# meteofrance/py4cast

Hardware: AMD Instinct MI355X
Metric: AR-training samples/sec (512x512x60 grid, 3-step rollout) (higher is better)
Workload: dtype bf16; 1 GPU; HalfUNet scaled_ar rollout T=3, grid 512x512x60 (+5 forcings, 4 statics), WeightedLoss(MSE), AdamW, B=2/GPU; global_batch=2, parallelism=dp1, border_size=0, setup_steps=2, accumulate_grad_batches=1, hip_graph=False, deterministic_library_solvers=False, full=False

## Files before the change

### include/py4cast_hip.h

```cpp
#ifndef PY4CAST_HIP_H
#define PY4CAST_HIP_H

#include <stddef.h>
#include <stdint.h>

#ifdef __cplusplus
extern "C" {
#endif

#define P4C_VERSION 100

typedef void* p4c_stream_t;

enum p4c_error {
    P4C_OK = 0,
    P4C_ERR_INVALID = -1,
    P4C_ERR_LAUNCH = -2,
    P4C_ERR_RUNTIME = -3,
    P4C_ERR_UNSUPPORTED = -4
};

enum p4c_dtype { P4C_F32 = 0, P4C_BF16 = 1 };

enum p4c_loss_kind { P4C_LOSS_MSE = 0, P4C_LOSS_L1 = 1 };
// ... 351 lines not shown
    int32_t cout;
    int32_t dx_channels;
    int32_t dtype;
    int32_t norm;
    int32_t groups;
    int32_t has_bias;
    float eps;
    float momentum;
    int32_t compute;
    int32_t weights_prepared;
    int32_t skip_out_conv;
} p4c_halfunet_desc;

int p4c_first_conv_tail_slots(int B, int H, int W);
int p4c_first_conv_tail(const void* x, int x_cs, int cin, const float* w, void* y, float* stat_partial, int B, int H, int W, p4c_stream_t stream);

int p4c_set_side_stream(p4c_stream_t side, void* const* events, int n_events);
int p4c_side_stream_defer(int on);
int p4c_side_stream_enable(int on);
long long p4c_side_stream_launch_count(void);
int p4c_side_stream_join(p4c_stream_t stream);
int p4c_graph_replace_memsets(void* graph, int* replaced, int* left);

int64_t p4c_halfunet_param_count(const p4c_halfunet_desc* d);
int p4c_halfunet_workspace_bytes(const p4c_halfunet_desc* d, size_t* saved_bytes, size_t* scratch_bytes);
typedef struct p4c_halfunet_layout_t {
    int64_t elem_bytes;
    int64_t Y[12], P[5], S, norm[12], saved_bytes;
    int64_t G0, TB, DY[2][12], k1[2][12], k2[2][12], scratch_bytes;
    int64_t w[12], gamma[12], beta[12], wout, params_bytes;
// ... 280 lines not shown
```

### py4cast_amd/_lib_model.py

```python

import ctypes
from ctypes import c_float, c_int, c_int32, c_int64, c_size_t, c_void_p

P, I, L, F = c_void_p, c_int, c_int64, c_float


class HalfUNetDesc(ctypes.Structure):

    _fields_ = [
        ("B", c_int32), ("H", c_int32), ("W", c_int32),
        ("cin", c_int32), ("cin_pad", c_int32), ("cout", c_int32), ("dx_channels", c_int32),
        ("dtype", c_int32), ("norm", c_int32), ("groups", c_int32), ("has_bias", c_int32),
        ("eps", c_float), ("momentum", c_float), ("compute", c_int32),
        ("weights_prepared", c_int32), ("skip_out_conv", c_int32),
    ]


DP = ctypes.POINTER(HalfUNetDesc)


class HalfUNetLayout(ctypes.Structure):

    _fields_ = [
        ("elem_bytes", c_int64),
# ... 28 lines not shown

SIGNATURES = {
    "p4c_prep_weights": [P, I, I, I, I, I, I, P, I, P],
    "p4c_conv_fwd": [P, I, I, I, P, I, P, P, I, P, P, I, P, I, I, I, I, P],
    "p4c_conv_wgrad": [P, I, I, I, I, P, P, I, P, I, I, P, P, I, I, I, P],
    "p4c_conv_small_fwd": [P, I, I, I, P, I, P, P, I, P, P, I, P, I, I, I, I, P, P, P, P, P, P, P, P, P, P, P, P, F, F, P, P, P, P, P, P,
                           P, P, P, P, P, P, P, P, P],
    "p4c_norm_finalize": [P, I, I, L, I, I, P, P, F, F, P, P, P, P, P, P, P],
    "p4c_conv_fwd_compact": [P, I, P, I, P, I, I, I, I, P],
    "p4c_conv_wgrad_compact": [P, I, I, P, I, I, I, P, P, I, I, I, P],
    "p4c_conv_wgrad_nb": [P, P, P, I, P, P, P, P, P, P, P, P, P, I, I, P, P, I, I, I, P],
    "p4c_conv_wgrad_kernel_kind": [I, I, I, I],
    "p4c_out_conv_bwd": [P, P, P, P, P, P, P, P, P, I, P, P, I, L, P],
    "p4c_upsample_sum_bwd_x": [I, P, I, I, I, P, P, P, P, P],
    "p4c_first_conv_tail": [P, I, I, P, P, P, I, I, I, P],
    "p4c_halfunet_workspace_bytes": [DP, ctypes.POINTER(c_size_t), ctypes.POINTER(c_size_t)],
    "p4c_halfunet_layout": [DP, ctypes.POINTER(HalfUNetLayout)],
    "p4c_halfunet_prepare_weights": [DP, P, P, P],
    "p4c_halfunet_forward": [DP, P, P, P, P, P, P, I, P],
    "p4c_halfunet_tail": [DP, P, P, P, P, P, P],
    "p4c_halfunet_backward": [DP, P, P, P, P, P, P, P, I, P],
    "p4c_side_stream_defer": [I],
    "p4c_side_stream_enable": [I],
    "p4c_side_stream_join": [P],
    "p4c_edge_gather_add_fwd": [P, P, P, P, P, P, L, I, I, I, P],
    "p4c_edge_gather_add_bwd": [P, P, P, P, P, P, P, L, I, I, I, P],
    "p4c_segment_sum": [P, P, P, P, P, L, L, I, I, I, P],
    "p4c_segment_sum_pair": [P, P, P, P, L, P, P, P, L, L, I, I, P],
    "p4c_row_layernorm_fwd": [P, P, P, P, F, P, L, I, I, P],
    "p4c_row_layernorm_bwd": [P, P, P, F, P, P, P, P, L, I, I, P],
# ... 55 lines not shown
    "p4c_deeplab_assemble_bwd": [P, P, P, P, P, I, I, I, P],
    "p4c_up2_cat_fwd": [P, P, P, L, I, I, I, I, I, P],
    "p4c_up2_cat_bwd": [P, L, P, P, I, I, I, I, I, P],
    "p4c_customunet_stem_fwd": [P, P, P, P, L, P, P, I, I, I, I, P],
    "p4c_customunet_stem_bwd": [P, P, L, P, P, P, P, P, P, P, P, I, I, I, I, P],
    "p4c_dlp_dw3x3_fwd": [P, P, P, P, P, I, I, I, I, I, I, I, I, P],
    "p4c_dlp_dw3x3_dgrad": [P, P, P, P, P, I, I, I, I, I, I, I, I, P],
    "p4c_dlp_dw3x3_wgrad": [P, P, P, P, P, I, I, I, I, I, I, I, I, P],
    "p4c_dlp_up_cat_fwd": [P, P, P, L, I, I, I, I, I, I, P],
    "p4c_dlp_up_cat_bwd": [P, L, P, P, I, I, I, I, I, I, P],
}
OTHER = {
    "p4c_conv_wgrad_workspace_bytes": ([I, I], c_size_t),
    "p4c_out_conv_bwd_slots": ([I, L], c_int),
    "p4c_first_conv_tail_slots": ([I, I, I], c_int),
    "p4c_out_conv_bwd_workspace_bytes": ([I, L], c_size_t),
    "p4c_conv_stat_tiles": ([I, I, I, I, I, I], c_int),
    "p4c_conv_stat_tiles_ks": ([I, I, I, I, I, I, I], c_int),
    "p4c_conv_kernel_kind": ([I, I, I, I, I, I, I], c_int),
    "p4c_conv_small_ok": ([I, I, I, I], c_int),
    "p4c_conv_small_stat_slots": ([I, I, I], c_int),
    "p4c_conv_compact_supported": ([I, I, I, I, I, I], c_int),
    "p4c_halfunet_param_count": ([DP], c_int64),
    "p4c_window_attn_bwd_workspace_bytes": ([I, I, I, I, I], c_size_t),
    "p4c_row_layernorm_bwd_workspace_bytes": ([L, I, I], c_size_t),
    "p4c_row_linear_wgrad_workspace_bytes": ([L, I], c_size_t),
    "p4c_row_gemm_supported": ([I, I], c_int),
    "p4c_row_gemm_wgrad_supported": ([I, I, I], c_int),
    "p4c_row_gemm_wgrad_workspace_bytes": ([L, I, I, I], c_size_t),
    "p4c_row_mlp_bwd_workspace_bytes": ([L, I], c_size_t),
# ... 17 lines not shown
```

### py4cast_amd/csrc/conv_bf16.hip

```cpp
#include <stdlib.h>

#include <type_traits>

#include "kernels.hpp"

namespace p4c {

typedef float f32x16 __attribute__((ext_vector_type(16)));
typedef float f32x4 __attribute__((ext_vector_type(4)));
typedef __bf16 bf16x8 __attribute__((ext_vector_type(8)));
typedef __bf16 bf16x4 __attribute__((ext_vector_type(4)));
typedef short s16x4 __attribute__((ext_vector_type(4)));

constexpr int BTW = 32;

#ifndef P4C_PRIO
#define P4C_PRIO 0
#endif
#ifndef P4C_EXP
#define P4C_EXP 0
#endif

#ifdef P4C_STAMPS
__device__ unsigned long long* g_stamps = nullptr;
// ... 2150 lines not shown
    if (blockIdx.x == 0 && blockIdx.y == 0 && (int)threadIdx.x < pb.n_zero) pb.zero_words[threadIdx.x] = 0u;
    const PrepJob& jb = pb.job[blockIdx.y];
    const int total = jb.M_pad * jb.K_pad * jb.ntaps;
    const int kv = pb.bf16 ? 8 : 4;
    const int ksteps = jb.K_pad / (2 * kv);
    for (int i = blockIdx.x * 256 + threadIdx.x; i < total; i += gridDim.x * 256) {
        int t = i;
        const int j = t % kv; t /= kv;
        const int m_l = t & 63; t >>= 6;
        const int h = t & 1; t >>= 1;
        const int ks = t % ksteps; t /= ksteps;
        const int tap = t % jb.ntaps;
        const int mb = t / jb.ntaps;
        const int k = 2 * kv * ks + kv * h + j, m = 64 * mb + m_l;
        float v = 0.0f;
        if (!jb.transpose_flip) {
            if (m < jb.CO && k < jb.CI) v = jb.w[((int64_t)m * jb.CI + k) * jb.ntaps + tap];
        } else {
            if (k < jb.CO && m < jb.CI) v = jb.w[((int64_t)k * jb.CI + m) * jb.ntaps + (jb.ntaps - 1 - tap)];
        }
        if (pb.bf16) reinterpret_cast<__bf16*>(jb.out)[i] = (__bf16)v;
        else reinterpret_cast<float*>(jb.out)[i] = v;
    }
}

int prep_weights_batch(const PrepBatch& pb, hipStream_t stream) {
    if (pb.n <= 0) return P4C_OK;
    int maxtotal = 0;
    for (int i = 0; i < pb.n; ++i) {
        const int t = pb.job[i].M_pad * pb.job[i].K_pad * pb.job[i].ntaps;
        if (t > maxtotal) maxtotal = t;
// ... 10 lines not shown
```

### py4cast_amd/csrc/conv_rows.hip

```cpp
#include <stddef.h>
#include <stdlib.h>

#include "kernels.hpp"

namespace p4c {

#ifndef P4C_EXP
#define P4C_EXP 0
#endif

#ifdef P4C_STAMPS
__device__ unsigned long long* g_rows_stamps = nullptr;
__device__ __forceinline__ void rows_stamp(int slot) {
    if (g_rows_stamps && blockIdx.x == 7 && blockIdx.y == 0 && blockIdx.z == 0 && (threadIdx.x & 63) == 0) {
        unsigned long long t;
        asm volatile("s_memtime %0\n\ts_waitcnt lgkmcnt(0)" : "=s"(t)::"memory");
        g_rows_stamps[2 * slot] = t;
        g_rows_stamps[2 * slot + 1] = __builtin_amdgcn_s_memrealtime();
    }
}
#define P4C_STAMP(slot) rows_stamp(slot)
#if P4C_STAMPS == 1
#define P4C_STAMP_ROW(slot) rows_stamp(slot)
#else
// ... 55 lines not shown
    const float ylo = __builtin_bit_cast(float, y2 << 16), yhi = __builtin_bit_cast(float, y2 & 0xffff0000u);
    const float glo = __builtin_fmaf(ylo, sc.x, sh.x) > 0.f ? __builtin_bit_cast(float, a2 << 16) : 0.f;
    const float ghi = __builtin_fmaf(yhi, sc.y, sh.y) > 0.f ? __builtin_bit_cast(float, a2 & 0xffff0000u) : 0.f;
    const float lo = __builtin_fmaf(al.x, glo, __builtin_fmaf(be.x, ylo, de.x));
    const float hi = __builtin_fmaf(al.y, ghi, __builtin_fmaf(be.y, yhi, de.y));
    const f32x2 v = {lo, hi};
    return __builtin_bit_cast(unsigned int, __builtin_convertvector(v, bf16x2));
}

__device__ __forceinline__ __amdgpu_buffer_rsrc_t make_rsrc(const void* base, unsigned int bytes) {
    return __builtin_amdgcn_make_buffer_rsrc(const_cast<void*>(base), 0, (int)bytes, 0x00020000);
}

__device__ __forceinline__ void lds_barrier() { asm volatile("s_waitcnt lgkmcnt(0)\n\ts_barrier" ::: "memory"); }

template <bool HP, bool HQ, bool HS>
__device__ __forceinline__ void conv_row(const bf16x8 (&A)[9][4], f32x16& P, f32x16& Q, f32x16& S, bf16x8 (&fb)[6],
                                         const char* rb, const char* rbn, bool pf, char* stg, const int (&soff)[4]) {
    using namespace rows;
    constexpr int PIXB = Lay<32>::PIXB;
    auto stage = [&](int g) __attribute__((always_inline)) {
        const f32x2 lo = {P[4 * g], P[4 * g + 1]}, hi = {P[4 * g + 2], P[4 * g + 3]};
        u32x2 o;
        o[0] = __builtin_bit_cast(unsigned int, __builtin_convertvector(lo, bf16x2));
        o[1] = __builtin_bit_cast(unsigned int, __builtin_convertvector(hi, bf16x2));
        *reinterpret_cast<u32x2*>(stg + soff[g]) = o;
    };
#pragma unroll
    for (int s = 0; s < 14; ++s) {
        const int o = s + 3;
        if (!(P4C_EXP & 16)) {
            if (o < 12) {
                fb[o % 6] = *reinterpret_cast<const bf16x8*>(rb + (o >> 2) * PIXB + (o & 3) * 32);
            } else if (o < 15) {
                if (pf) fb[o % 6] = *reinterpret_cast<const bf16x8*>(rbn + ((o - 12) >> 2) * PIXB + ((o - 12) & 3) * 32);
            }
            __builtin_amdgcn_sched_barrier(0);
            if (HP && s < 12) {
                P = __builtin_amdgcn_mfma_f32_32x32x16_bf16(A[6 + (s >> 2)][s & 3], fb[s % 6], P, 0, 0, 0);
                __builtin_amdgcn_sched_barrier(0);
            }
        }
        if (s >= 2) {
            const int q = s - 2;
            if (HQ && !(P4C_EXP & 16)) {
                Q = __builtin_amdgcn_mfma_f32_32x32x16_bf16(A[3 + (q >> 2)][q & 3], fb[q % 6], Q, 0, 0, 0);
                __builtin_amdgcn_sched_barrier(0);
            }
            if (HP && s >= 12) { stage(2 * (s - 12)); __builtin_amdgcn_sched_barrier(0); }
            if (HS && !(P4C_EXP & 16)) {
                if (q == 0) {
                    f32x16 z;
#pragma unroll
                    for (int i = 0; i < 16; ++i) z[i] = 0.f;
                    S = __builtin_amdgcn_mfma_f32_32x32x16_bf16(A[q >> 2][q & 3], fb[q % 6], z, 0, 0, 0);
                } else {
                    S = __builtin_amdgcn_mfma_f32_32x32x16_bf16(A[q >> 2][q & 3], fb[q % 6], S, 0, 0, 0);
                }
                __builtin_amdgcn_sched_barrier(0);
            }
            if (HP && s >= 12) { stage(2 * (s - 12) + 1); __builtin_amdgcn_sched_barrier(0); }
        }
    }
}

struct Acc16 { f32x4 v[2][2]; };

template <bool HP, bool HQ, bool HS>
__device__ __forceinline__ void conv_row16(const bf16x8 (&A)[9][2][2], Acc16& P, Acc16& Q, Acc16& S, bf16x8 (&fb)[6],
                                           int (&boff)[3][2], int delta, bool pf, const char* lring, char* stg,
                                           const int (&soff)[2]) {
    auto stage = [&](int mb, int nb) __attribute__((always_inline)) {
        const f32x4 a = P.v[mb][nb];
        const f32x2 lo = {a[0], a[1]}, hi = {a[2], a[3]};
        u32x2 o;
        o[0] = __builtin_bit_cast(unsigned int, __builtin_convertvector(lo, bf16x2));
// ... 55 lines not shown
    NormBwdCoef nb;
    BatchFin fin;
};
template <typename T>
__device__ __forceinline__ T late_arg(size_t offset) {
#if defined(__HIP_DEVICE_COMPILE__)
    const char* ka = (const char*)__builtin_amdgcn_kernarg_segment_ptr();
    asm volatile("" : "+s"(ka));
    return *reinterpret_cast<const T*>(ka + offset);
#else
    (void)offset;
    return T{};
#endif
}

template <int MODE, bool BST, int MF, int KS, bool CPT = false, int IV = 4>
__global__ void __launch_bounds__(512) __attribute__((amdgpu_waves_per_eu(2, 2)))
    conv3x3_bf16_rows_kernel(RowsArgs args) {
    static_assert(!CPT || (MODE == 0 && !BST && MF == 32), "compact channels: plain launches only");
    static_assert(IV == 4 || IV == 2, "rows per interval");
    using namespace rows;
    constexpr int NLD = (IV * ROWSLOTS + 255) / 256, NST = IV * 2;
    const __bf16* __restrict__ in = args.in;
    const __bf16* __restrict__ wp = args.wp;
    const float* __restrict__ in_scale = args.in_scale;
    const float* __restrict__ in_shift = args.in_shift;
    __bf16* __restrict__ out = args.out;
    float* __restrict__ stat_partial = args.stat_partial;
    const int out_cs = args.out_cs, H = args.H, W = args.W, rows_lo = args.rows_lo, rows_rem = args.rows_rem;
    const RingBwdStats& bst = args.bst;
    const NormBwdCoef& nb = args.nb;
    typedef Lay<MF> LY;
    constexpr int PIXB = LY::PIXB, RROW = LY::RROW, RINGB = LY::RINGB;
    extern __shared__ __attribute__((aligned(16))) char smem[];
    char* lring = smem;
    char* lstg = smem + RINGB;

// ... 2 lines not shown
    const int seg = blockIdx.x, strip = blockIdx.y, b = blockIdx.z;
    const int nseg = gridDim.x, nstrips = gridDim.y;
    const int wg_id = (b * nstrips + strip) * nseg + seg, wg_count = nseg * nstrips * gridDim.z;
    const int y0 = seg * rows_lo + (seg < rows_rem ? seg : rows_rem);
    const int R = rows_lo + (seg < rows_rem ? 1 : 0);
    const int x0 = strip * SW;
    const int K = (R + 2 + IV - 1) / IV;

    if (wv >= 4) {
        const int ltid = threadIdx.x - 256, lwv = wv - 4, c8 = ltid & 7;
        const int ipb = CPT ? args.in_cs * 2 : 128;
        const bool in_ch = !CPT || 8 * c8 < args.in_cs, out_ch = !CPT || 8 * c8 < out_cs;
        const __amdgpu_buffer_rsrc_t rs_in = make_rsrc(in + (int64_t)b * H * W * (ipb >> 1), (unsigned int)H * W * (unsigned int)ipb);
        const __amdgpu_buffer_rsrc_t rs_out = make_rsrc(out + (int64_t)b * H * W * out_cs, (unsigned int)H * W * out_cs * 2u);
        int gofs[NLD], lofs[NLD], lim[NLD];
        int rr = 0, rem = ltid;
#pragma unroll
        for (int it = 0; it < NLD; ++it) {
            const int idx = ltid + it * 256;
            if (it > 0) { rem += 256; if (rem >= ROWSLOTS) { rem -= ROWSLOTS; ++rr; } }
            const int col = rem >> 3;
            gofs[it] = in_ch ? (rr * W + col) * ipb + 16 * c8 : OOB;
            lofs[it] = rr * RROW + LY::slot_off(col, c8);
            lim[it] = ((unsigned)(x0 - 1 + col) < (unsigned)W) ? idx : OOB;
        }
        {
            const int left = x0 == 0 ? 1 : 0;
            const int c_hi = W - x0 + 1 < LW ? W - x0 + 1 : LW;
            const int ninv = left + (LW - c_hi);
            for (int rz = 0; rz < NR; ++rz)
                for (int j = ltid; j < ninv * 8; j += 256) {
                    const int s8 = j & 7, ci = j >> 3;
                    const int col = (left && ci == 0) ? 0 : c_hi + ci - left;
                    *reinterpret_cast<u32x4*>(lring + rz * RROW + col * PIXB + 16 * s8) = u32x4{0u, 0u, 0u, 0u};
                }
        }
        int dofs[NST], sofs[NST];
#pragma unroll
        for (int j = 0; j < NST; ++j) {
            const int px = (ltid + j * 256) >> 3, row = px >> 6, col = px & 63;
            dofs[j] = out_ch ? ((row * W + col) * out_cs + 8 * c8) * 2 : OOB;
            sofs[j] = row * SROW + col * 128 + ((c8 ^ ((col >> 1) & 7)) << 4);
        }
        f32x2 sc[4], sh[4], al[4], be[4], dl[4];
#pragma unroll
        for (int k = 0; k < 4; ++k) {
            sc[k] = sh[k] = al[k] = be[k] = dl[k] = f32x2{0.f, 0.f};
            if (MODE == 2 || MODE == 3) {
                sc[k] = *reinterpret_cast<const f32x2*>(in_scale + b * 64 + 8 * c8 + 2 * k);
// ... 19 lines not shown
            const int m0 = IV * k;
            int nrows = R + 2 - m0;
            nrows = nrows > IV ? IV : (nrows < 0 ? 0 : nrows);
            if ((P4C_EXP & 2) && k > 1) nrows = 0;
            const int nact = nrows * ROWSLOTS;
            const int gy0 = y0 - 1 + m0, gx0 = x0 - 1;
            if (gy0 >= 0 && gy0 + nrows <= H) {
                const int so = (gy0 * W + gx0) * ipb;
#pragma unroll
                for (int it = 0; it < NLD; ++it)
                    im.s[it] = __builtin_amdgcn_raw_buffer_load_b128(rs_in, (lim[it] < nact) ? gofs[it] : OOB, so, 0);
                if (MODE == 4) {
#pragma unroll
                    for (int it = 0; it < NLD; ++it)
                        ty.s[it] = __builtin_amdgcn_raw_buffer_load_b128(rs_nby, (lim[it] < nact) ? gofs[it] : OOB, so, 0);
                }
            } else {
#pragma unroll
                for (int it = 0; it < NLD; ++it) {
                    const int idx = ltid + it * 256, rr = idx / ROWSLOTS;
                    const int gy = gy0 + rr, gx = gx0 + ((idx - rr * ROWSLOTS) >> 3);
                    const bool ok = (idx < nact) & ((unsigned)gy < (unsigned)H) & ((unsigned)gx < (unsigned)W) & in_ch;
                    im.s[it] = __builtin_amdgcn_raw_buffer_load_b128(rs_in, ok ? (gy * W + gx) * ipb + 16 * c8 : OOB, 0, 0);
                    if (MODE == 4) ty.s[it] = __builtin_amdgcn_raw_buffer_load_b128(rs_nby, ok ? (gy * W + gx) * 128 + 16 * c8 : OOB, 0, 0);
                }
            }
        };
        auto store = [&](const Img& im, int k) __attribute__((always_inline)) {
            const int m0 = IV * k;
            int nrows = R + 2 - m0;
// ... 272 lines not shown
        {
            const char* wsrc = reinterpret_cast<const char*>(wp) + (h * 64 + ct * 32 + r) * 16;
#pragma unroll
            for (int tap = 0; tap < 9; ++tap)
#pragma unroll
                for (int ks = 0; ks < 4; ++ks) A[tap][ks] = *reinterpret_cast<const bf16x8*>(wsrc + (tap * 4 + ks) * 2048);
        }
        const int lane_base = (32 * ph + r) * PIXB + 16 * h;
        int soff[4];
#pragma unroll
        for (int g = 0; g < 4; ++g) soff[g] = (32 * ph + r) * 128 + 8 * h + (((4 * ct + g) ^ (((32 * ph + r) >> 1) & 7)) << 4);
        f32x16 a, bq, c;
#pragma unroll
        for (int i = 0; i < 16; ++i) a[i] = bq[i] = c[i] = 0.f;
        bf16x8 fb[6];
        auto rbase = [&](int mm) __attribute__((always_inline)) { return lring + (mm & 7) * RROW + lane_base; };
        auto issue3 = [&](const char* rb) __attribute__((always_inline)) {
            if (!(P4C_EXP & 16)) {
#pragma unroll
                for (int o = 0; o < 3; ++o) fb[o] = *reinterpret_cast<const bf16x8*>(rb + (o >> 2) * PIXB + (o & 3) * 32);
            }
        };
        if (wv == 0) P4C_STAMP(10);
        lds_barrier();
        if (wv == 0) P4C_STAMP(11);
        issue3(rbase(0));
#define P4C_ROW(HP, HQ, HS, P, Q, S)                                                                                        \
    {                                                                                                                       \
        const bool pf = ((m & (IV - 1)) != IV - 1) && (m != last);                                                          \
        if (wv == 0) P4C_STAMP_ROW(300 + 2 * m);                                                                            \
        conv_row<HP, HQ, HS>(A, P, Q, S, fb, rbase(m), rbase(m + 1), pf, lstg + (m & 7) * SROW, soff);                     \
        if (wv == 0) P4C_STAMP_ROW(301 + 2 * m);                                                                            \
        if (m == last) {                                                                                                    \
            P4C_STAMP(700 + 8 * (m >> 2) + 2 * wv);                                                                         \
            lds_barrier();                                                                                                  \
            P4C_STAMP(701 + 8 * (m >> 2) + 2 * wv);                                                                         \
        } else if ((m & (IV - 1)) == IV - 1) {                                                                              \
            P4C_STAMP(700 + 8 * (m >> 2) + 2 * wv);                                                                         \
            lds_barrier();                                                                                                  \
            P4C_STAMP(701 + 8 * (m >> 2) + 2 * wv);                                                                         \
            issue3(rbase(m + 1));                                                                                           \
        }                                                                                                                   \
        ++m;                                                                                                                \
    }
        P4C_ROW(false, false, true, a, a, a)
        P4C_ROW(false, true, true, a, a, bq)
// ... 79 lines not shown
#define P4C_ROTATE() { const Acc16 t_ = a; a = bq; bq = c; c = t_; }
        while (m < R) {
            P4C_ROW(true, true, true, a, bq, c)
            P4C_ROTATE()
        }
        P4C_ROW(true, true, false, a, bq, a)
        P4C_ROTATE()
        P4C_ROW(true, false, false, a, a, a)
#undef P4C_ROTATE
#undef P4C_ROW
        if (P4C_EXP & 16) { asm volatile("" ::"v"(A[0][0][0]), "v"(A[8][1][1])); }
    }
    if (wv == 0) P4C_STAMP(12);
}

static int rows_mfma_shape() {
    const char* e = diag_env("P4C_ROWS_MFMA");
    return (e && atoi(e) == 16) ? 16 : 32;
}

template <int MODE, bool BST, int KS, int IV = 4>
int launch_rows_mode(const __bf16* in, const __bf16* wp, const float* in_scale, const float* in_shift, __bf16* out, int out_cs,
                     float* stat_partial, int B, int H, int W, int nstrips, int nseg, hipStream_t stream, const BatchFin& fin,
                     const RingBwdStats& bst, const NormBwdCoef& nb = NormBwdCoef{}) {
    const RowsArgs args{in, wp, in_scale, in_shift, out, stat_partial, out_cs, H, W, H / nseg, H % nseg, fin.slots ? 1 : 0, 64, bst, nb, fin};
    if (KS == 1 || MODE == 4 || rows_mfma_shape() == 32) {
        P4C_TRY(ensure_dyn_smem((const void*)conv3x3_bf16_rows_kernel<MODE, BST, 32, KS, false, IV>, rows::Lay<32>::SMEM));
        hipLaunchKernelGGL((conv3x3_bf16_rows_kernel<MODE, BST, 32, KS, false, IV>), dim3(nseg, nstrips, B), dim3(512), rows::Lay<32>::SMEM, stream, args);
    } else if (KS == 3 && MODE != 4) {
        constexpr int M16 = MODE == 4 ? 0 : MODE;
// ... 81 lines not shown
    const int rc = ks == 3 ? launch_rows_compact<3>((const __bf16*)in, in_cs, (const __bf16*)wp, (__bf16*)out, out_cs, B, H, W, nstrips, nseg, stream)
                           : launch_rows_compact<1>((const __bf16*)in, in_cs, (const __bf16*)wp, (__bf16*)out, out_cs, B, H, W, nstrips, nseg, stream);
    if (rc != P4C_OK) return rc;
    P4C_CHECK_LAUNCH("conv_bf16_rows_compact");
    return P4C_OK;
}

int launch_conv_bf16_rows_wide_pixels(const void* in, int pixel_channels, const void* wp, void* out, int B, int H, int W, hipStream_t stream) {
    if (pixel_channels < 64 || pixel_channels % 8 || !conv_bf16_is_rows(P4C_BF16, 64, 3, 1, 64, B, H, W) ||
        (int64_t)H * W * pixel_channels * 2 >= (int64_t)1 << 31)
        return fail(P4C_ERR_UNSUPPORTED, "conv_bf16_rows_wide_pixels: unsupported shape (%d-channel pixels, %dx%dx%d)", pixel_channels, B, H, W);
    int nstrips, nseg;
    conv_rows_geometry(B, H, W, &nstrips, &nseg);
    const int rc = launch_rows_compact<3>((const __bf16*)in, pixel_channels, (const __bf16*)wp, (__bf16*)out, 64, B, H, W, nstrips, nseg, stream);
    if (rc != P4C_OK) return rc;
    P4C_CHECK_LAUNCH("conv_bf16_rows_wide_pixels");
    return P4C_OK;
}

int conv_rows_stat_slots(int B, int H, int W) {
    int nstrips, nseg;
    conv_rows_geometry(B, H, W, &nstrips, &nseg);
    return nstrips * nseg * 4;
}

int launch_conv3x3_bf16_rows(const void* inv, const void* wpv, int ks, const float* in_scale, const float* in_shift, int in_relu,
                             void* outv, int out_cs, float* stat_partial, int B, int H, int W, hipStream_t stream, const BatchFin* finp,
                             const RingBwdStats* bst, int* nblk_out, const NormBwdCoef* nb) {
    const __bf16* in = (const __bf16*)inv;
    const __bf16* wp = (const __bf16*)wpv;
    __bf16* out = (__bf16*)outv;
// ... 27 lines not shown
```

### py4cast_amd/csrc/conv_thin.hip

```cpp
#include <stdlib.h>

#include "kernels.hpp"

namespace p4c {
namespace {

typedef float f32x16 __attribute__((ext_vector_type(16)));
typedef float f32x4 __attribute__((ext_vector_type(4)));
typedef __bf16 bf16x8 __attribute__((ext_vector_type(8)));
typedef unsigned int u32x4 __attribute__((ext_vector_type(4)));

constexpr int OOB = 0x7fffffff;
constexpr int SP = 68;
constexpr int WIMG_BYTES = 2 * 5 * 64 * 16;

struct ThinArgs {
    const __bf16* x;
    const float* w;
    __bf16* y;
    float* stat_partial;
    int x_cs, c0, nc, cin;
    int H, W, nblk;
};

// ... 115 lines not shown
    if (n > 256) n = 256;
    const int64_t cap = 2 * (int64_t)num_cus() / (B > 0 ? B : 1);
    if (n > cap && cap >= 1) n = cap;
    return n < 1 ? 1 : (int)n;
}

}

bool first_conv_split_ok(int compute, int storage, int cin, int cin_pad, int B, int H, int W) {
    const char* e = diag_env("P4C_FIRST_CONV_SPLIT");
    if (e && e[0] == '0') return false;
    return compute == P4C_BF16 && storage == P4C_BF16 && cin_pad == 96 && cin > 64 && cin <= 72 && W % 32 == 0 &&
           conv_bf16_is_rows(storage, 64, 3, 1, 64, B, H, W) && (int64_t)H * W * 192 < ((int64_t)1 << 31);
}

int first_conv_tail_slots(int B, int H, int W) { return tail_blocks(B, H, W) * 4; }

int launch_first_conv_tail(const void* x, int x_cs, int cin, const float* w, void* y, float* stat_partial, int B, int H, int W, hipStream_t stream) {
    ThinArgs a{(const __bf16*)x, w, (__bf16*)y, stat_partial, x_cs, 64, cin - 64, cin, H, W, tail_blocks(B, H, W)};
    hipLaunchKernelGGL(first_conv_tail_kernel, dim3(a.nblk, B), dim3(256), 0, stream, a);
    P4C_CHECK_LAUNCH("first_conv_tail");
    return P4C_OK;
}

namespace {
namespace wt {
constexpr int SW = 64, LW = SW + 2;
constexpr int RPI = 2;
constexpr int NRX = 8, NRD = 2 * RPI;
constexpr int XROW = LW * 16, DROW = SW * 128;
constexpr int XRING = NRX * XROW, DRING = NRD * DROW;
constexpr int SLAB = 9 * 8 * 64;
__device__ __forceinline__ int slot_off(int col, int c8) { return col * 128 + ((((c8 >> 2) ^ (col >> 1)) & 1) << 6) + ((c8 & 3) << 4); }
}

// ... 177 lines not shown
    P4C_CHECK_LAUNCH("conv3x3_wgrad_thin_bf16");
    *nslots_out = nwg;
    return P4C_OK;
}

}

extern "C" int p4c_first_conv_tail_slots(int B, int H, int W) { return p4c::first_conv_tail_slots(B, H, W); }
extern "C" int p4c_first_conv_tail(const void* x, int x_cs, int cin, const float* w, void* y, float* stat_partial, int B, int H, int W,
                                   p4c_stream_t stream) {
    P4C_CHECK_ARG(x && w && y, "p4c_first_conv_tail: NULL pointer");
    P4C_CHECK_ARG(cin > 64 && cin <= 72 && x_cs >= 72 && x_cs % 8 == 0 && W % 32 == 0 && B > 0 && H > 0,
                  "p4c_first_conv_tail: 65..72 input channels on pixels of >= 72 channels (multiple of 8), W a multiple of 32");
    return p4c::launch_first_conv_tail(x, x_cs, cin, w, y, stat_partial, B, H, W, p4c::as_stream(stream));
}
```

### py4cast_amd/csrc/halfunet.cpp

```cpp
#include <stdlib.h>

#include <atomic>
#include <functional>
#include <vector>

#include "kernels.hpp"

namespace p4c {
namespace {

constexpr int NF = 64;
constexpr int NLEV = 5;
constexpr int NCONV = 12;
constexpr int NWSLOT = 2 * NCONV + 3;

constexpr int64_t HANDOFF_SLOT_FLOATS = 256 * 128;

struct Layout {
    int esz;
    int64_t n[NLEV];
    int Hk[NLEV], Wk[NLEV];
    int64_t w[NCONV], gamma[NCONV], beta[NCONV], wout, nparams;
    int64_t Y[NCONV], P[NLEV], S, act_elems, norm_base, norm[NCONV], saved_bytes;
    int64_t wslot_floats;
// ... 150 lines not shown
}

inline void* wslot(const WS& ws, int slot) { return ws.f(ws.L.wprep + (int64_t)slot * ws.L.wslot_floats); }

int prepare_weights(const p4c_halfunet_desc& d, const WS& ws, const float* params, int which, hipStream_t st) {
    const Layout& L = ws.L;
    PrepBatch pb;
    pb.n = 0;
    pb.bf16 = d.compute == P4C_BF16;
    for (int i = 0; i < NCONV; ++i) {
        if (which & 1) pb.job[pb.n++] = {params + L.w[i], wslot(ws, i), NF, conv_cin(d, i), 9, 0, 64, conv_cin_pad(d, i)};
        if (which & 2) pb.job[pb.n++] = {params + L.w[i], wslot(ws, NCONV + i), NF, conv_cin(d, i), 9, 1, i == 0 ? 64 * dx_blocks(d) : 64, NF};
    }
    if (which & 1) pb.job[pb.n++] = {params + L.wout, wslot(ws, 2 * NCONV), d.cout, NF, 1, 0, 64, NF};
    if ((which & 1) && first_conv_split_ok(d.compute, d.dtype, d.cin, d.cin_pad, d.B, d.H, d.W))
        pb.job[pb.n++] = {params + L.w[0], wslot(ws, 2 * NCONV + 2), NF, d.cin, 9, 0, 64, NF};
    if (which & 2) pb.job[pb.n++] = {params + L.wout, wslot(ws, 2 * NCONV + 1), d.cout, NF, 1, 1, 64, NF};
    pb.zero_words = reinterpret_cast<unsigned int*>(ws.f(L.tickets));
    pb.n_zero = 64;
    return prep_weights_batch(pb, st);
}

bool small_handoff(const p4c_halfunet_desc& d, const Layout& L, int lev, int training) {
    const char* ie = diag_env("P4C_NO_INKERNEL_FINALIZE");
    return lev > 0 && training && d.norm == 0 && d.compute == P4C_BF16 && !(ie && ie[0] == '1') &&
           conv_small_handoff_ok(d.dtype, d.B, L.Hk[lev], L.Wk[lev]);
}

int conv_block_fwd(const p4c_halfunet_desc& d, const WS& ws, int i, const void* in, const Norm* in_norm, const float* params,
                   float* running, int training, hipStream_t st, int handoff = 0) {
    const Layout& L = ws.L;
// ... 21 lines not shown
    if (small) {
        float* other = statp ? statp + HANDOFF_SLOT_FLOATS : nullptr;
        BatchFin pre{};
        if (handoff == 2) {
            Norm pn = norm_at(ws, i - 1, d.B);
            float* prm = running ? running + (int64_t)(i - 1) * 128 : nullptr;
            pre = BatchFin{other, nullptr, params + L.gamma[i - 1], params + L.beta[i - 1], prm, prm ? prm + 64 : nullptr,
                           pn.scale, pn.shift, pn.mean, pn.rstd, (double)d.B * H * W, d.eps, d.momentum, d.B};
        }
        const bool given = in_norm && handoff != 2;
        P4C_TRY(launch_conv3x3_bf16_small(in, wp, given ? in_norm->scale : nullptr, given ? in_norm->shift : nullptr, in_norm ? 1 : 0,
                                          ws.act(L.Y[i]), handoff == 1 ? other : statp, d.B, H, W, st,
                                          infin && handoff != 1 ? &fin : nullptr, handoff == 2 ? &pre : nullptr));
        if (handoff == 1) return P4C_OK;
        ntiles = conv_small_stat_slots(d.B, H, W);
    } else if (i == 0 && !in_norm && first_conv_split_ok(d.compute, d.dtype, d.cin, d.cin_pad, d.B, H, W)) {
        P4C_TRY(launch_conv_bf16_rows_wide_pixels(in, d.cin_pad, wslot(ws, 2 * NCONV + 2), ws.act(L.Y[i]), d.B, H, W, st));
        P4C_TRY(launch_first_conv_tail(in, d.cin_pad, d.cin, params + L.w[0], ws.act(L.Y[i]), statp, d.B, H, W, st));
        ntiles = first_conv_tail_slots(d.B, H, W);
    } else {
        P4C_TRY(conv_fwd(d.compute, d.dtype, in, conv_cin_pad(d, i), wp, 3, in_norm ? in_norm->scale : nullptr,
                         in_norm ? in_norm->shift : nullptr, in_norm ? 1 : 0, ws.act(L.Y[i]), NF, statp, d.B, H, W, 1, st,
                         infin ? &fin : nullptr));
    }
    if (infin) return P4C_OK;
    if (batch_stats) {
        P4C_TRY(norm_finalize(statp, ntiles, d.B, (int64_t)H * W, d.norm,
                              d.groups, params + L.gamma[i], params + L.beta[i], d.eps, d.momentum,
                              d.norm == 0 ? rm : nullptr, d.norm == 0 ? rv : nullptr, nm.scale, nm.shift, nm.mean, nm.rstd, st));
    } else {
// ... 613 lines not shown
```

### py4cast_amd/csrc/kernels.hpp

```cpp
#pragma once
#include "common.hpp"

namespace p4c {

int prep_weights(const float* w, int CO, int CI, int ks, int transpose_flip, int M_pad, int K_pad, float* out,
                 hipStream_t stream);
int conv_fwd_f32(const float* in, int CI, const float* wp, int ks, const float* in_scale, const float* in_shift,
                 int in_relu, const float* bias, float* out, int out_cs, float* stat_partial, int B, int H, int W,
                 int m_blocks, hipStream_t stream);
int conv_wgrad_f32(const float* in, int CI, int ks, const float* in_scale, const float* in_shift, int in_relu,
                   const float* dout, float* partial, int G, int B, int H, int W, int CO, int CIreal, float* grad,
                   hipStream_t stream);
static inline int64_t wgrad_partial_floats(int CI_pad, int ks, int G) { return (int64_t)2 * G * ks * ks * CI_pad * 64; }

int wgrad_reduce(const float* partial, int nslots, int ks, int CI_pad, int ci_lo, int ci_hi, int CO, int CI, float* grad,
                 hipStream_t stream, int ci_base = 0);
struct WgradReduceJob {
    const float* partial;
    float* grad;
    int nslots, ntaps, CI_pad, ci_lo, ci_hi, CO, CI;
    int ci_base = 0;
};
constexpr int WGRAD_BATCH_MAX = 24;
struct WgradCollect {
    WgradReduceJob job[WGRAD_BATCH_MAX];
    int n = 0;
};
void wgrad_collect_into(WgradCollect* c);
int wgrad_reduce_batch(const WgradCollect& c, hipStream_t stream);

int prep_weights_bf16(const float* w, int CO, int CI, int ks, int transpose_flip, int M_pad, int K_pad, void* out,
                      hipStream_t stream);
struct PrepJob {
    const float* w;
    void* out;
    int CO, CI, ntaps, transpose_flip, M_pad, K_pad;
};
struct PrepBatch {
    PrepJob job[32];
    int n;
    int bf16;
    unsigned int* zero_words;
    int n_zero;
};

struct BatchFin {
    float* slots;
    unsigned int* ticket;
    const float* gamma;
    const float* beta;
    float* running_mean;
// ... 72 lines not shown
bool conv_wgrad_bf16_takes_nb(int storage, int CI, int ks, int B);
bool conv_rows_compact_ok(int storage, int in_cs, int out_cs, int ks, int B, int H, int W);
int launch_conv_bf16_rows_compact(const void* in, int in_cs, const void* wp, int ks, void* out, int out_cs, int B, int H, int W,
                                  hipStream_t stream);
int conv_wgrad_bf16_compact(const void* in, int in_cs, int ks, const void* dout, int dout_cs, float* partial, int G, int B, int H, int W,
                            int CO, int CIreal, float* grad, hipStream_t stream);

bool first_conv_split_ok(int compute, int storage, int cin, int cin_pad, int B, int H, int W);
int first_conv_tail_slots(int B, int H, int W);
int launch_first_conv_tail(const void* x, int x_cs, int cin, const float* w, void* y, float* stat_partial, int B, int H, int W, hipStream_t stream);
bool conv_wgrad_thin_ok(int storage, int in_cs, int ci_real, int dout_cs, int ks, int B, int H, int W);
int conv_wgrad_thin_slots(int G, int B, int H, int W, int* nseg_out = nullptr);
int launch_conv3x3_wgrad_thin_bf16(const void* x, int in_cs, const void* dout, float* partial, int G, int B, int H, int W, hipStream_t stream,
                                   int* nslots_out);
int launch_conv_bf16_rows_wide_pixels(const void* in, int pixel_channels, const void* wp, void* out, int B, int H, int W, hipStream_t stream);

int norm_finalize(const float* partial, int tiles_per_sample, int B, int64_t hw, int mode, int groups, const float* gamma,
                  const float* beta, float eps, float momentum, float* running_mean, float* running_var, float* scale,
                  float* shift, float* mean, float* rstd, hipStream_t stream);
int norm_eval(int B, const float* gamma, const float* beta, float eps, const float* running_mean,
              const float* running_var, float* scale, float* shift, float* mean, float* rstd, hipStream_t stream);
int norm_bwd_blocks(int64_t hw);
int norm_bwd(int storage, const void* dA, const void* y, const float* scale, const float* shift, const float* mean,
             const float* rstd, const float* gamma, int relu, int B, int64_t hw, int mode, int groups, int training,
             float* partial, float* k1, float* k2, float* dgamma, float* dbeta, void* dY, hipStream_t stream, int pre_nblk = 0,
             unsigned int* fin_ticket = nullptr, bool pre_finalized = false);
constexpr int NORM_BWD_MAX_BLOCKS = 1024;
int pool_fwd(int storage, const void* y, const float* scale, const float* shift, int B, int H, int W, void* P,
             hipStream_t stream);
int upsum_fwd(int storage, const void* const* y, const float* const* scale, const float* const* shift, int B, int H, int W,
// ... 28 lines not shown
```

Baseline: 457.3 samples/s.

## Fold first-conv tail channels into the rows MFMA kernel as a ninth octet

Adds a thin variant of the compact 3x3 rows conv kernel that also loads the ninth 8-channel octet of input pixels and runs extra MFMAs on a packed weight image, so the first HalfUNet conv (65..72 input channels) runs in a single launch. Previously it ran as a wide-pixel rows conv over 64 channels plus a separate tail kernel that re-read the input and accumulated the rest. Weight prep gains a thin packing mode and extra LDS is reserved for the tail weights. This removes one launch and a second pass over input and output, at the cost of more LDS, more registers and a longer per-row schedule in the hot kernel. The new path is taken by default and can be disabled through an environment variable.

```diff
diff --git a/include/py4cast_hip.h b/include/py4cast_hip.h
--- a/include/py4cast_hip.h
+++ b/include/py4cast_hip.h
@@ -389,6 +389,10 @@
 
 int p4c_first_conv_tail_slots(int B, int H, int W);
 int p4c_first_conv_tail(const void* x, int x_cs, int cin, const float* w, void* y, float* stat_partial, int B, int H, int W, p4c_stream_t stream);
+int p4c_first_conv_one_slots(int B, int H, int W);
+int p4c_first_conv_one(const void* x, int x_cs, int cin, const float* w, void* y, float* stat_partial, int B, int H, int W, p4c_stream_t stream);
+int p4c_first_conv_two(const void* x, int x_cs, int cin, const float* w, void* y, float* stat_partial, int B, int H, int W, p4c_stream_t stream);
+long long p4c_first_conv_launch_count(void);
 
 int p4c_set_side_stream(p4c_stream_t side, void* const* events, int n_events);
 int p4c_side_stream_defer(int on);
diff --git a/py4cast_amd/_lib_model.py b/py4cast_amd/_lib_model.py
--- a/py4cast_amd/_lib_model.py
+++ b/py4cast_amd/_lib_model.py
@@ -66,6 +66,8 @@
     "p4c_out_conv_bwd": [P, P, P, P, P, P, P, P, P, I, P, P, I, L, P],
     "p4c_upsample_sum_bwd_x": [I, P, I, I, I, P, P, P, P, P],
     "p4c_first_conv_tail": [P, I, I, P, P, P, I, I, I, P],
+    "p4c_first_conv_one": [P, I, I, P, P, P, I, I, I, P],
+    "p4c_first_conv_two": [P, I, I, P, P, P, I, I, I, P],
     "p4c_halfunet_workspace_bytes": [DP, ctypes.POINTER(c_size_t), ctypes.POINTER(c_size_t)],
     "p4c_halfunet_layout": [DP, ctypes.POINTER(HalfUNetLayout)],
     "p4c_halfunet_prepare_weights": [DP, P, P, P],
@@ -151,6 +153,8 @@
     "p4c_conv_wgrad_workspace_bytes": ([I, I], c_size_t),
     "p4c_out_conv_bwd_slots": ([I, L], c_int),
     "p4c_first_conv_tail_slots": ([I, I, I], c_int),
+    "p4c_first_conv_one_slots": ([I, I, I], c_int),
+    "p4c_first_conv_launch_count": ([], ctypes.c_longlong),
     "p4c_out_conv_bwd_workspace_bytes": ([I, L], c_size_t),
     "p4c_conv_stat_tiles": ([I, I, I, I, I, I], c_int),
     "p4c_conv_stat_tiles_ks": ([I, I, I, I, I, I, I], c_int),
diff --git a/py4cast_amd/csrc/conv_bf16.hip b/py4cast_amd/csrc/conv_bf16.hip
--- a/py4cast_amd/csrc/conv_bf16.hip
+++ b/py4cast_amd/csrc/conv_bf16.hip
@@ -2188,7 +2188,10 @@
         const int mb = t / jb.ntaps;
         const int k = 2 * kv * ks + kv * h + j, m = 64 * mb + m_l;
         float v = 0.0f;
-        if (!jb.transpose_flip) {
+        if (jb.thin) {
+            const int ky = tap >> 1, kx = 2 * (tap & 1) + h;
+            if (kx < 3 && m < jb.CO && 64 + j < jb.CI) v = jb.w[((int64_t)m * jb.CI + 64 + j) * 9 + 3 * ky + kx];
+        } else if (!jb.transpose_flip) {
             if (m < jb.CO && k < jb.CI) v = jb.w[((int64_t)m * jb.CI + k) * jb.ntaps + tap];
         } else {
             if (k < jb.CO && m < jb.CI) v = jb.w[((int64_t)k * jb.CI + m) * jb.ntaps + (jb.ntaps - 1 - tap)];
diff --git a/py4cast_amd/csrc/conv_rows.hip b/py4cast_amd/csrc/conv_rows.hip
--- a/py4cast_amd/csrc/conv_rows.hip
+++ b/py4cast_amd/csrc/conv_rows.hip
@@ -93,11 +93,14 @@
 
 __device__ __forceinline__ void lds_barrier() { asm volatile("s_waitcnt lgkmcnt(0)\n\ts_barrier" ::: "memory"); }
 
-template <bool HP, bool HQ, bool HS>
+template <bool HP, bool HQ, bool HS, bool THIN = false>
 __device__ __forceinline__ void conv_row(const bf16x8 (&A)[9][4], f32x16& P, f32x16& Q, f32x16& S, bf16x8 (&fb)[6],
-                                         const char* rb, const char* rbn, bool pf, char* stg, const int (&soff)[4]) {
+                                         const char* rb, const char* rbn, bool pf, char* stg, const int (&soff)[4],
+                                         const char* tw = nullptr, int tl0 = 0, int tl1 = 0) {
     using namespace rows;
     constexpr int PIXB = Lay<32>::PIXB;
+    bf16x8 tb[2], ta[2];
+    auto thin_has = [](int j) { return j % 3 == 0 ? HP : (j % 3 == 1 ? HQ : HS); };
     auto stage = [&](int g) __attribute__((always_inline)) {
         const f32x2 lo = {P[4 * g], P[4 * g + 1]}, hi = {P[4 * g + 2], P[4 * g + 3]};
         u32x2 o;
@@ -114,6 +117,12 @@
             } else if (o < 15) {
                 if (pf) fb[o % 6] = *reinterpret_cast<const bf16x8*>(rbn + ((o - 12) >> 2) * PIXB + ((o - 12) & 3) * 32);
             }
+            if constexpr (THIN) {
+                if (s == 3) tb[0] = *reinterpret_cast<const bf16x8*>(rb + tl0);
+                if (s == 6) tb[1] = *reinterpret_cast<const bf16x8*>(rb + tl1);
+                if (s >= 3 && s < 9 && thin_has(s - 3))
+                    ta[(s - 3) & 1] = *reinterpret_cast<const bf16x8*>(tw + ((2 - (s - 3) % 3) * 2 + (s - 3) / 3) * 2048);
+            }
             __builtin_amdgcn_sched_barrier(0);
             if (HP && s < 12) {
                 P = __builtin_amdgcn_mfma_f32_32x32x16_bf16(A[6 + (s >> 2)][s & 3], fb[s % 6], P, 0, 0, 0);
@@ -139,6 +148,14 @@
                 __builtin_amdgcn_sched_barrier(0);
             }
             if (HP && s >= 12) { stage(2 * (s - 12) + 1); __builtin_amdgcn_sched_barrier(0); }
+        }
+        if constexpr (THIN) {
+            if (s >= 4 && s < 10 && thin_has(s - 4) && !(P4C_EXP & 16)) {
+                const int j = s - 4;
+                f32x16& T = j % 3 == 0 ? P : (j % 3 == 1 ? Q : S);
+                T = __builtin_amdgcn_mfma_f32_32x32x16_bf16(ta[j & 1], tb[j / 3], T, 0, 0, 0);
+                __builtin_amdgcn_sched_barrier(0);
+            }
         }
     }
 }
@@ -224,13 +241,13 @@
 #endif
 }
 
-template <int MODE, bool BST, int MF, int KS, bool CPT = false, int IV = 4>
-__global__ void __launch_bounds__(512) __attribute__((amdgpu_waves_per_eu(2, 2)))
-    conv3x3_bf16_rows_kernel(RowsArgs args) {
+template <int MODE, bool BST, int MF, int KS, bool CPT, int IV, bool THIN>
+__device__ __forceinline__ void conv3x3_bf16_rows_body(const RowsArgs& args) {
     static_assert(!CPT || (MODE == 0 && !BST && MF == 32), "compact channels: plain launches only");
+    static_assert(!THIN || (CPT && KS == 3 && IV == 4), "ninth channel octet: a compact 3x3 launch");
     static_assert(IV == 4 || IV == 2, "rows per interval");
     using namespace rows;
-    constexpr int NLD = (IV * ROWSLOTS + 255) / 256, NST = IV * 2;
+    constexpr int NLD = (IV * ROWSLOTS + (THIN ? IV * LW : 0) + 255) / 256, NST = IV * 2;
     const __bf16* __restrict__ in = args.in;
     const __bf16* __restrict__ wp = args.wp;
     const float* __restrict__ in_scale = args.in_scale;
@@ -263,6 +280,26 @@
         const __amdgpu_buffer_rsrc_t rs_in = make_rsrc(in + (int64_t)b * H * W * (ipb >> 1), (unsigned int)H * W * (unsigned int)ipb);
         const __amdgpu_buffer_rsrc_t rs_out = make_rsrc(out + (int64_t)b * H * W * out_cs, (unsigned int)H * W * out_cs * 2u);
         int gofs[NLD], lofs[NLD], lim[NLD];
+        auto thin_slot = [&](int it, int& row, int& col, int& oct) __attribute__((always_inline)) {
+            const int idx = ltid + it * 256;
+            if (idx < IV * ROWSLOTS) {
+                row = idx / ROWSLOTS; col = (idx - row * ROWSLOTS) >> 3; oct = c8;
+                return true;
+            }
+            const int p = idx - IV * ROWSLOTS;
+            row = p / LW; col = p - row * LW; oct = 8;
+            return p < IV * LW;
+        };
+        if constexpr (THIN) {
+#pragma unroll
+            for (int it = 0; it < NLD; ++it) {
+                int row, col, oct;
+                const bool ex = thin_slot(it, row, col, oct);
+                gofs[it] = ex ? (row * W + col) * ipb + 16 * oct : OOB;
+                lofs[it] = row * RROW + col * PIXB + 16 * oct;
+                lim[it] = (ex && (unsigned)(x0 - 1 + col) < (unsigned)W) ? row * ROWSLOTS + col * 8 + (oct & 7) : OOB;
+            }
+        } else {
         int rr = 0, rem = ltid;
 #pragma unroll
         for (int it = 0; it < NLD; ++it) {
@@ -272,6 +309,7 @@
             gofs[it] = in_ch ? (rr * W + col) * ipb + 16 * c8 : OOB;
             lofs[it] = rr * RROW + LY::slot_off(col, c8);
             lim[it] = ((unsigned)(x0 - 1 + col) < (unsigned)W) ? idx : OOB;
+        }
         }
         {
             const int left = x0 == 0 ? 1 : 0;
@@ -282,6 +320,7 @@
                     const int s8 = j & 7, ci = j >> 3;
                     const int col = (left && ci == 0) ? 0 : c_hi + ci - left;
                     *reinterpret_cast<u32x4*>(lring + rz * RROW + col * PIXB + 16 * s8) = u32x4{0u, 0u, 0u, 0u};
+                    if (THIN && s8 == 0) *reinterpret_cast<u32x4*>(lring + rz * RROW + col * PIXB + 128) = u32x4{0u, 0u, 0u, 0u};
                 }
         }
         int dofs[NST], sofs[NST];
@@ -331,6 +370,15 @@
 #pragma unroll
                     for (int it = 0; it < NLD; ++it)
                         ty.s[it] = __builtin_amdgcn_raw_buffer_load_b128(rs_nby, (lim[it] < nact) ? gofs[it] : OOB, so, 0);
+                }
+            } else if constexpr (THIN) {
+#pragma unroll
+                for (int it = 0; it < NLD; ++it) {
+                    int row, col, oct;
+                    const bool ex = thin_slot(it, row, col, oct);
+                    const int gy = gy0 + row, gx = gx0 + col;
+                    const bool ok = ex & (row < nrows) & ((unsigned)gy < (unsigned)H) & ((unsigned)gx < (unsigned)W);
+                    im.s[it] = __builtin_amdgcn_raw_buffer_load_b128(rs_in, ok ? (gy * W + gx) * ipb + 16 * oct : OOB, 0, 0);
                 }
             } else {
 #pragma unroll
@@ -633,6 +681,15 @@
 #pragma unroll
         for (int i = 0; i < 16; ++i) a[i] = bq[i] = c[i] = 0.f;
         bf16x8 fb[6];
+        const char* tw = nullptr;
+        const int tl0 = h * PIXB + 128 - 16 * h, tl1 = (2 - h) * PIXB + 128 - 16 * h;
+        if constexpr (THIN) {
+            char* lthin = lstg + STGB;
+            const u32x4* src = reinterpret_cast<const u32x4*>(wp + 9 * 64 * 64);
+#pragma unroll
+            for (int j = 0; j < 3; ++j) *reinterpret_cast<u32x4*>(lthin + (threadIdx.x + 256 * j) * 16) = src[threadIdx.x + 256 * j];
+            tw = lthin + (h * 64 + ct * 32 + r) * 16;
+        }
         auto rbase = [&](int mm) __attribute__((always_inline)) { return lring + (mm & 7) * RROW + lane_base; };
         auto issue3 = [&](const char* rb) __attribute__((always_inline)) {
             if (!(P4C_EXP & 16)) {
@@ -648,7 +705,7 @@
     {                                                                                                                       \
         const bool pf = ((m & (IV - 1)) != IV - 1) && (m != last);                                                          \
         if (wv == 0) P4C_STAMP_ROW(300 + 2 * m);                                                                            \
-        conv_row<HP, HQ, HS>(A, P, Q, S, fb, rbase(m), rbase(m + 1), pf, lstg + (m & 7) * SROW, soff);                     \
+        conv_row<HP, HQ, HS, THIN>(A, P, Q, S, fb, rbase(m), rbase(m + 1), pf, lstg + (m & 7) * SROW, soff, tw, tl0, tl1); \
         if (wv == 0) P4C_STAMP_ROW(301 + 2 * m);                                                                            \
         if (m == last) {                                                                                                    \
             P4C_STAMP(700 + 8 * (m >> 2) + 2 * wv);                                                                         \
@@ -758,6 +815,18 @@
     if (wv == 0) P4C_STAMP(12);
 }
 
+template <int MODE, bool BST, int MF, int KS, bool CPT = false, int IV = 4>
+__global__ void __launch_bounds__(512) __attribute__((amdgpu_waves_per_eu(2, 2)))
+    conv3x3_bf16_rows_kernel(RowsArgs args) {
+    conv3x3_bf16_rows_body<MODE, BST, MF, KS, CPT, IV, false>(args);
+}
+
+constexpr int THIN_IMG_BYTES = 3 * 2 * 2 * 64 * 16;
+__global__ void __launch_bounds__(512) __attribute__((amdgpu_waves_per_eu(2, 2)))
+    conv3x3_bf16_rows_thin_kernel(RowsArgs args) {
+    conv3x3_bf16_rows_body<0, false, 32, 3, true, 4, true>(args);
+}
+
 static int rows_mfma_shape() {
     const char* e = diag_env("P4C_ROWS_MFMA");
     return (e && atoi(e) == 16) ? 16 : 32;
@@ -869,7 +938,29 @@
     conv_rows_geometry(B, H, W, &nstrips, &nseg);
     const int rc = launch_rows_compact<3>((const __bf16*)in, pixel_channels, (const __bf16*)wp, (__bf16*)out, 64, B, H, W, nstrips, nseg, stream);
     if (rc != P4C_OK) return rc;
+    count_first_conv_launch();
     P4C_CHECK_LAUNCH("conv_bf16_rows_wide_pixels");
+    return P4C_OK;
+}
+
+size_t first_conv_one_image_bytes() { return (size_t)9 * 64 * 64 * 2 + THIN_IMG_BYTES; }
+bool first_conv_one_ok(int pixel_channels, int B, int H, int W) {
+    return pixel_channels >= 72 && pixel_channels % 8 == 0 && conv_bf16_is_rows(P4C_BF16, 64, 3, 1, 64, B, H, W) &&
+           (int64_t)H * W * pixel_channels * 2 < (int64_t)1 << 31;
+}
+int launch_first_conv_one(const void* in, int pixel_channels, const void* wp, void* out, float* stat_partial, int B, int H, int W,
+                          hipStream_t stream) {
+    if (!first_conv_one_ok(pixel_channels, B, H, W))
+        return fail(P4C_ERR_UNSUPPORTED, "first_conv_one: unsupported shape (%d-channel pixels, %dx%dx%d)", pixel_channels, B, H, W);
+    int nstrips, nseg;
+    conv_rows_geometry(B, H, W, &nstrips, &nseg);
+    const RowsArgs args{(const __bf16*)in, (const __bf16*)wp, nullptr, nullptr, (__bf16*)out, stat_partial, 64, H, W, H / nseg, H % nseg, 0,
+                        pixel_channels, RingBwdStats{}, NormBwdCoef{}, BatchFin{}};
+    constexpr int smem = rows::Lay<32>::SMEM + THIN_IMG_BYTES;
+    P4C_TRY(ensure_dyn_smem((const void*)conv3x3_bf16_rows_thin_kernel, smem));
+    hipLaunchKernelGGL(conv3x3_bf16_rows_thin_kernel, dim3(nseg, nstrips, B), dim3(512), smem, stream, args);
+    count_first_conv_launch();
+    P4C_CHECK_LAUNCH("first_conv_one");
     return P4C_OK;
 }
 
diff --git a/py4cast_amd/csrc/conv_thin.hip b/py4cast_amd/csrc/conv_thin.hip
--- a/py4cast_amd/csrc/conv_thin.hip
+++ b/py4cast_amd/csrc/conv_thin.hip
@@ -1,4 +1,6 @@
 #include <stdlib.h>
+
+#include <atomic>
 
 #include "kernels.hpp"
 
@@ -153,11 +155,22 @@
            conv_bf16_is_rows(storage, 64, 3, 1, 64, B, H, W) && (int64_t)H * W * 192 < ((int64_t)1 << 31);
 }
 
+bool first_conv_one_routed(int compute, int storage, int cin, int cin_pad, int B, int H, int W) {
+    const char* e = diag_env("P4C_FIRST_CONV_ONE");
+    if (e && e[0] == '0') return false;
+    return first_conv_split_ok(compute, storage, cin, cin_pad, B, H, W) && first_conv_one_ok(cin_pad, B, H, W);
+}
+
 int first_conv_tail_slots(int B, int H, int W) { return tail_blocks(B, H, W) * 4; }
+
+static std::atomic<long long> g_first_conv_launches{0};
+void count_first_conv_launch() { g_first_conv_launches.fetch_add(1); }
+long long first_conv_launches() { return g_first_conv_launches.load(); }
 
 int launch_first_conv_tail(const void* x, int x_cs, int cin, const float* w, void* y, float* stat_partial, int B, int H, int W, hipStream_t stream) {
     ThinArgs a{(const __bf16*)x, w, (__bf16*)y, stat_partial, x_cs, 64, cin - 64, cin, H, W, tail_blocks(B, H, W)};
     hipLaunchKernelGGL(first_conv_tail_kernel, dim3(a.nblk, B), dim3(256), 0, stream, a);
+    count_first_conv_launch();
     P4C_CHECK_LAUNCH("first_conv_tail");
     return P4C_OK;
 }
@@ -365,3 +378,47 @@
                   "p4c_first_conv_tail: 65..72 input channels on pixels of >= 72 channels (multiple of 8), W a multiple of 32");
     return p4c::launch_first_conv_tail(x, x_cs, cin, w, y, stat_partial, B, H, W, p4c::as_stream(stream));
 }
+
+namespace p4c {
+namespace {
+int first_conv_single_op(bool one, const void* x, int x_cs, int cin, const float* w, void* y, float* stat_partial, int B, int H, int W,
+                         hipStream_t st) {
+    void* img = nullptr;
+    P4C_CHECK_HIP(hipMallocAsync(&img, first_conv_one_image_bytes(), st));
+    PrepBatch pb;
+    pb.n = 0;
+    pb.bf16 = 1;
+    pb.zero_words = nullptr;
+    pb.n_zero = 0;
+    pb.job[pb.n++] = {w, img, 64, cin, 9, 0, 64, 64};
+    if (one) pb.job[pb.n++] = {w, (char*)img + 9 * 64 * 64 * 2, 64, cin, 6, 0, 64, 16, 1};
+    int rc = prep_weights_batch(pb, st);
+    if (rc == P4C_OK) {
+        if (one) {
+            rc = launch_first_conv_one(x, x_cs, img, y, stat_partial, B, H, W, st);
+        } else {
+            rc = launch_conv_bf16_rows_wide_pixels(x, x_cs, img, y, B, H, W, st);
+            if (rc == P4C_OK) rc = launch_first_conv_tail(x, x_cs, cin, w, y, stat_partial, B, H, W, st);
+        }
+    }
+    (void)hipFreeAsync(img, st);
+    return rc;
+}
+}
+}
+extern "C" long long p4c_first_conv_launch_count(void) { return p4c::first_conv_launches(); }
+extern "C" int p4c_first_conv_one_slots(int B, int H, int W) { return p4c::conv_rows_stat_slots(B, H, W); }
+extern "C" int p4c_first_conv_one(const void* x, int x_cs, int cin, const float* w, void* y, float* stat_partial, int B, int H, int W,
+                                  p4c_stream_t stream) {
+    P4C_CHECK_ARG(x && w && y, "p4c_first_conv_one: NULL pointer");
+    P4C_CHECK_ARG(cin > 64 && cin <= 72 && x_cs >= 72 && x_cs % 8 == 0 && W % 32 == 0 && B > 0 && H > 0,
+                  "p4c_first_conv_one: 65..72 input channels on pixels of >= 72 channels (multiple of 8), W a multiple of 32");
+    return p4c::first_conv_single_op(true, x, x_cs, cin, w, y, stat_partial, B, H, W, p4c::as_stream(stream));
+}
+extern "C" int p4c_first_conv_two(const void* x, int x_cs, int cin, const float* w, void* y, float* stat_partial, int B, int H, int W,
+                                  p4c_stream_t stream) {
+    P4C_CHECK_ARG(x && w && y, "p4c_first_conv_two: NULL pointer");
+    P4C_CHECK_ARG(cin > 64 && cin <= 72 && x_cs >= 72 && x_cs % 8 == 0 && W % 32 == 0 && B > 0 && H > 0,
+                  "p4c_first_conv_two: 65..72 input channels on pixels of >= 72 channels (multiple of 8), W a multiple of 32");
+    return p4c::first_conv_single_op(false, x, x_cs, cin, w, y, stat_partial, B, H, W, p4c::as_stream(stream));
+}
diff --git a/py4cast_amd/csrc/halfunet.cpp b/py4cast_amd/csrc/halfunet.cpp
--- a/py4cast_amd/csrc/halfunet.cpp
+++ b/py4cast_amd/csrc/halfunet.cpp
@@ -188,7 +188,11 @@
     }
     if (which & 1) pb.job[pb.n++] = {params + L.wout, wslot(ws, 2 * NCONV), d.cout, NF, 1, 0, 64, NF};
     if ((which & 1) && first_conv_split_ok(d.compute, d.dtype, d.cin, d.cin_pad, d.B, d.H, d.W))
+    {
         pb.job[pb.n++] = {params + L.w[0], wslot(ws, 2 * NCONV + 2), NF, d.cin, 9, 0, 64, NF};
+        if (first_conv_one_ok(d.cin_pad, d.B, d.H, d.W))
+            pb.job[pb.n++] = {params + L.w[0], static_cast<char*>(wslot(ws, 2 * NCONV + 2)) + 9 * 64 * NF * 2, NF, d.cin, 6, 0, 64, 16, 1};
+    }
     if (which & 2) pb.job[pb.n++] = {params + L.wout, wslot(ws, 2 * NCONV + 1), d.cout, NF, 1, 1, 64, NF};
     pb.zero_words = reinterpret_cast<unsigned int*>(ws.f(L.tickets));
     pb.n_zero = 64;
@@ -240,6 +244,9 @@
                                           infin && handoff != 1 ? &fin : nullptr, handoff == 2 ? &pre : nullptr));
         if (handoff == 1) return P4C_OK;
         ntiles = conv_small_stat_slots(d.B, H, W);
+    } else if (i == 0 && !in_norm && first_conv_one_routed(d.compute, d.dtype, d.cin, d.cin_pad, d.B, H, W)) {
+        P4C_TRY(launch_first_conv_one(in, d.cin_pad, wslot(ws, 2 * NCONV + 2), ws.act(L.Y[i]), statp, d.B, H, W, st));
+        ntiles = conv_rows_stat_slots(d.B, H, W);
     } else if (i == 0 && !in_norm && first_conv_split_ok(d.compute, d.dtype, d.cin, d.cin_pad, d.B, H, W)) {
         P4C_TRY(launch_conv_bf16_rows_wide_pixels(in, d.cin_pad, wslot(ws, 2 * NCONV + 2), ws.act(L.Y[i]), d.B, H, W, st));
         P4C_TRY(launch_first_conv_tail(in, d.cin_pad, d.cin, params + L.w[0], ws.act(L.Y[i]), statp, d.B, H, W, st));
diff --git a/py4cast_amd/csrc/kernels.hpp b/py4cast_amd/csrc/kernels.hpp
--- a/py4cast_amd/csrc/kernels.hpp
+++ b/py4cast_amd/csrc/kernels.hpp
@@ -35,6 +35,7 @@
     const float* w;
     void* out;
     int CO, CI, ntaps, transpose_flip, M_pad, K_pad;
+    int thin = 0;
 };
 struct PrepBatch {
     PrepJob job[32];
@@ -137,6 +138,12 @@
 int launch_conv3x3_wgrad_thin_bf16(const void* x, int in_cs, const void* dout, float* partial, int G, int B, int H, int W, hipStream_t stream,
                                    int* nslots_out);
 int launch_conv_bf16_rows_wide_pixels(const void* in, int pixel_channels, const void* wp, void* out, int B, int H, int W, hipStream_t stream);
+bool first_conv_one_ok(int pixel_channels, int B, int H, int W);
+bool first_conv_one_routed(int compute, int storage, int cin, int cin_pad, int B, int H, int W);
+size_t first_conv_one_image_bytes();
+void count_first_conv_launch();
+int launch_first_conv_one(const void* in, int pixel_channels, const void* wp, void* out, float* stat_partial, int B, int H, int W,
+                          hipStream_t stream);
 
 int norm_finalize(const float* partial, int tiles_per_sample, int B, int64_t hw, int mode, int groups, const float* gamma,
                   const float* beta, float eps, float momentum, float* running_mean, float* running_var, float* scale,
```

Measured after the change: 470.6 samples/s (median of 6 runs). 2.9% higher.
